# widkyyu/Goal-conditioned-Reinforcement-Learning-with-environmental-and-policy-priors

Hardware: AMD Instinct MI355X
Metric: env-steps/sec (higher is better)
Workload: dtype u8

## Files before the change

goal-conditioned-reinforcement-learning-with-environmental-and-policy-priors_amd/_lib.py:

```python
import ctypes as C
import os
import subprocess

_PKG_DIR = os.path.dirname(os.path.abspath(__file__))
LIB_PATH = os.path.join(_PKG_DIR, "libtwoarmy_hip.so")
CSRC_DIR = os.path.join(_PKG_DIR, "csrc")

TW_CELLS = 289
TW_REC_WORDS = 48
TW_DRAW_WORDS = 8
TW_F_AUTORESET = 1
TW_F_POLICY_IDX = 2
TW_F_MATRIX_CODE = 4
TW_F_SLAB_HIPMALLOC = 8

FIELDS = dict(AX=0, AY=1, DIR=2, STEP_COUNT=3, STEP_MOVE=4, PONE=5, PATROL=6, UP1=7, RIGHT2=8, UPD_LONG=9,
              UPD_HORIZ=10, RISK=11, FIRST_ROOM2=12, OBX=13, OBY=16, O1X=19, O1Y=22, O1_VALID=25, O2X=26,
              O2Y=30, O2_VALID=34, GOAL_X=35, GOAL_Y=36, T=37, ERROR=38, MAX_STEPS=39, EPISODES=40,
              LAST_REWARD=41, LAST_TERM=42, LAST_TRUNC=43, WALL_I1=44, WALL_I2=45)

LAUNCH_FIELDS = ("pipelined", "PG", "LAYOUT", "pipe_grid", "E", "FAST", "seq_grid", "T")

ENV_ERRORS = {1: AttributeError, 2: AssertionError, 3: TypeError}

# ... 105 lines not shown
    "mg_nav_path_scan": (C.c_int, [_vp, _i64, _i, _i, _i, _i, _vp, _vp, _vp, _vp, _vp, _vp, _i, _vp, _vp, _vp, _vp, _vp, _vp,
                                   _vp, _vp, _vp]),
    "mg_nav_path_summary_workspace": (C.c_int, [_i, _i]),
    "mg_nav_path_summary": (C.c_int, [_vp, _vp, _vp, _vp, _vp, _vp, _i, _i, _vp, _vp, _vp]),
    "ppo_her_relabel": (C.c_int, [_vp, _vp, _vp, _vp, _vp, _vp, _u64, C.c_uint32, C.c_uint32, _i, _i, _i, _vp, _vp, _vp,
                                  _vp, _vp, _vp, _vp, _vp]),
    "ppo_her_relabel_window": (C.c_int, [_vp, _vp, _vp, _vp, _vp, _vp, _u64, C.c_uint32, C.c_uint32, _i, _i, _i, _i, _vp,
                                         _vp, _vp, _vp, _vp, _vp, _vp, _vp]),
    "ppo_lstm_cell": (C.c_int, [_vp, _vp, C.c_longlong, _vp, _vp, _vp, _i, _i, _vp]),
    "ppo_decoder_frames": (C.c_int, [_vp, _i, _vp, _vp, _vp, _vp, _vp, C.c_float, _vp, _vp]),
    "ppo_gather_stack_u8": (C.c_int, [_vp, _i, _vp, _i, _vp, _vp, _vp, _vp, _vp, _i, _vp, _vp, _vp]),
    "ppo_age_scan": (C.c_int, [_vp, _vp, _vp, _i, _i, _vp, _vp]),
    "ppo_episode_scan": (C.c_int, [_vp, _vp, _vp, _i, _i, _vp, _vp, _vp, _vp, _vp]),
    "ppo_episode_summary": (C.c_int, [_vp, _vp, _vp, _vp, _vp, _vp, _i, _i, _i, C.c_double, C.c_double, _vp, _vp, _vp, _vp,
                                      _vp, _vp]),
    "ppo_episode_summary_workspace": (C.c_int, [_i, _i]),
    "ppo_visit_scan": (C.c_int, [_vp, _vp, _vp, _i, _i, _i, _i, _vp, _vp, _vp, _vp]),
    "ppo_visit_carry_words": (C.c_int, [_i, _i, _i]),
    "ppo_visit_hist": (C.c_int, [_vp, _i, _i, _vp, _vp, _vp, _i, _i, _i, _vp, _vp]),
    "ppo_bonus_table_words": (C.c_int, [_i, _i, _i, _i, _i, _i]),
    "ppo_bonus_workspace_bytes": (_i64, [_i, _i, _i, _i, _i, _i]),
    "ppo_bonus_scan": (C.c_int, [_vp, _vp, _vp, C.c_long, C.c_long, _vp, _vp, _i, _i, _i, _i, _i, _i, _i, C.c_double, _vp, _vp,
                                 _vp, _vp, _vp, _vp, _vp]),
    "ppo_bonus_episode_words": (C.c_int, [_i, _i, _i, _i, _i]),
    "ppo_bonus_scan_episode": (C.c_int, [_vp, _vp, _vp, C.c_long, C.c_long, _vp, _vp, _vp, _vp, _i, _i, _i, _i, _i, _i, _i,
                                         C.c_double, _vp, _vp, _vp, _vp, _vp, _vp]),
    "ppo_bias_relu_nhwc": (C.c_int, [_vp, _vp, _i64, _i, _vp]),
    "ppo_conv1_up4_bias_relu": (C.c_int, [_vp, _i, _i, _vp, _vp, _vp, _vp]),
    "ppo_conv1_up4_bias_relu_c": (C.c_int, [_vp, _i, _i, _i, _vp, _vp, _vp, _vp]),
    "ppo_conv1_up4_bwd_groups": (C.c_int, [_i]),
    "ppo_conv1_up4_bwd": (C.c_int, [_vp, _i, _i, _vp, _vp, _vp, _vp, _vp]),
    "ppo_relu_bwd_bias_grad_nhwc_blocks": (C.c_int, [_i64, _i]),
    "ppo_relu_bwd_bias_grad_nhwc": (C.c_int, [_vp, _vp, _vp, _vp, _i64, _i, _vp]),
})

_lib = None


def exported_symbols():
    return sorted(_SIGS)


def lib():
    global _lib
    if _lib is None:
        if not os.path.exists(LIB_PATH):
            raise TwoarmyLibraryError(
                "%s not built: run `python -c 'import __graft_entry__ as g; g.build()'` "
                "(hipcc --offload-arch=gfx950); there is no CPU fallback" % LIB_PATH)
        import torch
        try:
            h = C.CDLL(LIB_PATH)
        except OSError as ex:
            raise TwoarmyLibraryError("cannot load %s: %s" % (LIB_PATH, ex)) from ex
        for name, (res, args) in _SIGS.items():
            try:
                fn = getattr(h, name)
            except AttributeError as ex:
                raise TwoarmyLibraryError("%s lacks symbol %s" % (LIB_PATH, name)) from ex
            fn.restype, fn.argtypes = res, args
        runtimes = set()
        try:
            with open("/proc/self/maps") as f:
                for line in f:
                    if "libamdhip64" in line:
                        runtimes.add(line.split()[-1])
# ... 17 lines not shown
```

goal-conditioned-reinforcement-learning-with-environmental-and-policy-priors_amd/csrc/ppo_kernels.hip:

```cpp

#include <hip/hip_runtime.h>
#include <float.h>
#include <stdint.h>

#include <type_traits>

#include "launch.h"
#include "philox.h"
#include "twoarmy.h"
#include "twoarmy_ppo.h"

namespace {

constexpr float CAT_EPS = FLT_EPSILON;

template <int A> __device__ __forceinline__ float cat_row(const float *__restrict__ row, float (&p)[A]) {
    float S = 0.f;
#pragma unroll
    for (int k = 0; k < A; ++k) { p[k] = row[k]; S += p[k]; }
    return S;
}
__device__ __forceinline__ float cat_log(float q) { return logf(fminf(fmaxf(q, CAT_EPS), 1.0f - CAT_EPS)); }

template <typename T, int K> __device__ __forceinline__ void block_sum(T (&v)[K], T *lds) {
    const int tid = threadIdx.x;
#pragma unroll
    for (int k = 0; k < K; ++k) lds[k * 256 + tid] = v[k];
    __syncthreads();
    for (int s = 128; s > 0; s >>= 1) {
        if (tid < s) {
#pragma unroll
            for (int k = 0; k < K; ++k) lds[k * 256 + tid] += lds[k * 256 + tid + s];
        }
        __syncthreads();
    }
#pragma unroll
    for (int k = 0; k < K; ++k) v[k] = lds[k * 256];
}

__device__ __forceinline__ float4 relu4(float4 v) {
    return make_float4(fmaxf(v.x, 0.f), fmaxf(v.y, 0.f), fmaxf(v.z, 0.f), fmaxf(v.w, 0.f));
}
__device__ __forceinline__ float4 mask4(float4 g, float4 y) {
    return make_float4(y.x > 0.f ? g.x : 0.f, y.y > 0.f ? g.y : 0.f, y.z > 0.f ? g.z : 0.f, y.w > 0.f ? g.w : 0.f);
}
__device__ __forceinline__ void add4(float4 &acc, const float4 &o) { acc.x += o.x; acc.y += o.y; acc.z += o.z; acc.w += o.w; }
__device__ __forceinline__ float4 fma4(float x, float4 w, float4 acc) {
    return make_float4(fmaf(x, w.x, acc.x), fmaf(x, w.y, acc.y), fmaf(x, w.z, acc.z), fmaf(x, w.w, acc.w));
}

__device__ __forceinline__ float4 slot_sum4(const float4 *red, int rows, int stride, int cq) {
    float4 sum = red[cq];
    for (int r = 1; r < rows; ++r) add4(sum, red[r * stride + cq]);
    return sum;
}

__device__ __forceinline__ uint32_t done_at(const uint8_t *__restrict__ terminated, const uint8_t *__restrict__ truncated,
                                            size_t i) {
    return (uint32_t)(terminated[i] | truncated[i]);
}

template <int A>
__global__ void ppo_sample_kernel(const float *__restrict__ probs, int B, const float *__restrict__ uniforms,
                                  uint32_t k0, uint32_t k1, uint64_t offset, const uint64_t *__restrict__ offset_dev,
                                  int32_t *__restrict__ action, float *__restrict__ logp) {
    const int b = blockIdx.x * blockDim.x + threadIdx.x;
    if (b >= B) return;
    float p[A];
    const float sum = cat_row<A>(probs + (size_t)b * A, p);
    float u;
    if (uniforms) u = uniforms[b];
    else {
        const uint64_t ctr = (uint64_t)b + offset + (offset_dev ? *offset_dev : 0ull);
        uint32_t c0 = (uint32_t)ctr, c1 = (uint32_t)(ctr >> 32), c2 = 0, c3 = 0x54574F53u;
        philox4x32_10(k0, k1, c0, c1, c2, c3);
        u = (float)(c0 >> 8) * (1.0f / 16777216.0f);
    }
    int a = A - 1, last = A - 1;
    float cum = 0.f, qa = 0.f;
    bool found = false;
#pragma unroll
    for (int k = 0; k < A; ++k) {
        const float q = p[k] / sum;
        cum += q;
        if (q > 0.f) last = k;
        if (!found && cum > u) { a = k; found = true; }
    }
    if (!found) a = last;
#pragma unroll
    for (int k = 0; k < A; ++k) if (k == a) qa = p[k] / sum;
    action[b] = a;
    logp[b] = cat_log(qa);
}

__global__ __launch_bounds__(256) void ppo_bias_relu_kernel(float4 *__restrict__ y, const float4 *__restrict__ bias,
                                                            size_t n4, int c4) {
    const size_t stride = (size_t)gridDim.x * blockDim.x;
    for (size_t i = (size_t)blockIdx.x * blockDim.x + threadIdx.x; i < n4; i += stride) {
        float4 v = y[i];
        add4(v, bias[i % c4]);
        y[i] = relu4(v);
    }
}

__global__ __launch_bounds__(256) void ppo_relu_bwd_bias_grad_kernel(const float4 *__restrict__ gy,
                                                                     const float4 *__restrict__ y,
                                                                     float4 *__restrict__ gx,
                                                                     float4 *__restrict__ partial, size_t n_pixels,
                                                                     int c4, int pixels_per_block) {
    __shared__ float4 red[256];
    const int rows = 256 / c4;
    const int cq = threadIdx.x % c4, row = threadIdx.x / c4;
    const size_t p0 = (size_t)blockIdx.x * pixels_per_block;
    const size_t p1 = p0 + pixels_per_block < n_pixels ? p0 + pixels_per_block : n_pixels;
    float4 acc = make_float4(0.f, 0.f, 0.f, 0.f);
    if (row < rows) {
        for (size_t px = p0 + row; px < p1; px += rows) {
            const size_t i = px * c4 + cq;
            const float4 o = mask4(gy[i], y[i]);
            gx[i] = o;
            add4(acc, o);
        }
    }
    red[threadIdx.x] = acc;
    __syncthreads();
    if (row == 0) partial[(size_t)blockIdx.x * c4 + cq] = slot_sum4(red, rows, c4, cq);
}

template <int F> __device__ __forceinline__ void conv1_stage_frame(float *xs, const float *__restrict__ src, int tid) {
    for (int i = tid; i < F * 324; i += 256) {
        const int c = i / 324, r = i - c * 324, y = r / 18, x = r - y * 18;
        xs[i] = (y < 17 && x < 17) ? src[c * 289 + y * 17 + x] : 0.f;
    }
}

template <int F, int CQ>
__global__ __launch_bounds__(256) void ppo_conv1_up4_kernel(const float *__restrict__ frames, const float4 *__restrict__ wf,
                                                            const float4 *__restrict__ bias, float4 *__restrict__ out, int B) {
    __shared__ float xs[F * 18 * 18];
    constexpr int SLOTS = 256 / CQ;
    const int b = blockIdx.x, tid = threadIdx.x;
    const int cq = tid % CQ, slot = tid / CQ;
    conv1_stage_frame<F>(xs, frames + (size_t)b * F * 289, tid);
    __syncthreads();
    const float4 bv = bias[cq];
    float4 *dst = out + (size_t)b * 1089 * CQ;
#pragma unroll 1
    for (int ph = 0; ph < 4; ++ph) {
        const int py = ph >> 1, px = ph & 1;
        float4 w[4 * F];
#pragma unroll
        for (int k = 0; k < 4 * F; ++k) w[k] = wf[(ph * 4 * F + k) * CQ + cq];
        const int ny = 17 - py, nx = 17 - px;
        for (int q = slot; q < ny * nx; q += SLOTS) {
            const int m = q / nx, n = q - m * nx;
            float4 acc = bv;
#pragma unroll
            for (int t = 0; t < 4; ++t) {
                const int ty = t >> 1, tx = t & 1;
#pragma unroll
                for (int c = 0; c < F; ++c) acc = fma4(xs[c * 324 + (m + ty) * 18 + n + tx], w[t * F + c], acc);
            }
            dst[((2 * m + py) * 33 + 2 * n + px) * CQ + cq] = relu4(acc);
        }
    }
}

template <int F>
__global__ __launch_bounds__(256) void ppo_conv1_up4_bwd_kernel(const float *__restrict__ frames, const float4 *__restrict__ gy,
                                                                const float4 *__restrict__ y, float4 *__restrict__ gw_part,
                                                                float4 *__restrict__ gb_part, int B) {
    __shared__ float xs[F * 18 * 18];
    __shared__ float4 red[256];
    const int tid = threadIdx.x, cq = tid & 15, slot = tid >> 4;
    const int ph = blockIdx.y, py = ph >> 1, px = ph & 1;
    const int ny = 17 - py, nx = 17 - px;
    float4 acc[4 * F];
#pragma unroll
    for (int k = 0; k < 4 * F; ++k) acc[k] = make_float4(0.f, 0.f, 0.f, 0.f);
    float4 accb = make_float4(0.f, 0.f, 0.f, 0.f);
    for (int b = blockIdx.x; b < B; b += gridDim.x) {
        __syncthreads();
        conv1_stage_frame<F>(xs, frames + (size_t)b * F * 289, tid);
        __syncthreads();
        const size_t base = (size_t)b * 1089 * 16;
        for (int q = slot; q < ny * nx; q += 16) {
            const int m = q / nx, n = q - m * nx;
            const size_t o = base + (size_t)((2 * m + py) * 33 + 2 * n + px) * 16 + cq;
            const float4 g = mask4(gy[o], y[o]);
            add4(accb, g);
#pragma unroll
            for (int t = 0; t < 4; ++t) {
                const int ty = t >> 1, tx = t & 1;
#pragma unroll
                for (int c = 0; c < F; ++c) acc[t * F + c] = fma4(xs[c * 324 + (m + ty) * 18 + n + tx], g, acc[t * F + c]);
            }
        }
    }
    const size_t wbase = ((size_t)blockIdx.x * 4 + ph) * (4 * F) * 16;
#pragma unroll
    for (int k = 0; k <= 4 * F; ++k) {
        __syncthreads();
        red[tid] = k < 4 * F ? acc[k < 4 * F ? k : 0] : accb;
        __syncthreads();
        if (slot == 0) {
            const float4 sum = slot_sum4(red, 16, 16, cq);
            if (k < 4 * F) gw_part[wbase + (size_t)k * 16 + cq] = sum;
            else gb_part[((size_t)blockIdx.x * 4 + ph) * 16 + cq] = sum;
        }
    }
}

constexpr int GT = 64;

template <int GN>
__global__ __launch_bounds__(256) void ppo_gae_kernel(const float *__restrict__ reward, const float *__restrict__ value,
                                                      const float *__restrict__ next_value,
                                                      const uint8_t *__restrict__ done, float gamma, float lambda,
                                                      int use_done_mask, int T, int N, float *__restrict__ adv,
                                                      float *__restrict__ target, float *__restrict__ ret) {
    __shared__ float sd[GT][GN + 1];
    __shared__ float sc[GT][GN + 1];
// ... 1156 lines not shown
    if (!all_set(reward, terminated, truncated, carry_return, carry_length) || T <= 0 || N <= 0 ||
        !ep_count_ok((int64_t)T * N) || !aligned_natural(reward, carry_return, carry_length, ep_return, ep_length))
        return TW_E_ARG;
    hipLaunchKernelGGL(ppo_episode_scan_kernel, dim3(blocks(N, 64)), dim3(64), 0, (hipStream_t)stream, reward, terminated,
                       truncated, T, N, carry_return, carry_length, ep_return, ep_length);
    return tw_launched(__func__);
}

int ppo_episode_summary_workspace(int T, int N) {
    if (T <= 0 || N <= 0 || !ep_count_ok((int64_t)T * N)) return TW_E_ARG;
    return ep_summary_blocks((int64_t)T * N) * EP_NV;
}

int ppo_episode_summary(const double *ep_return, const int32_t *ep_length, const uint8_t *terminated,
                        const uint8_t *truncated, const float *reward, const int32_t *action, int A, int T, int N,
                        double keep, double gain, double *score, double *summary, int64_t *action_hist,
                        int64_t *reward_hist, double *workspace, void *stream) {
    if (!all_set(ep_return, ep_length, terminated, truncated, reward, summary, reward_hist, workspace) || T <= 0 || N <= 0 ||
        !ppo_actions_ok(A) || !ep_count_ok((int64_t)T * N) ||
        !aligned_natural(ep_return, ep_length, reward, action, score, summary, action_hist, reward_hist, workspace))
        return TW_E_ARG;
    const int64_t M = (int64_t)T * N;
    const int nblocks = ep_summary_blocks(M);
    const int64_t per_block = (M + nblocks - 1) / nblocks;
    const int per_thread = blocks(per_block, 256);
    hipStream_t st = (hipStream_t)stream;
    hipLaunchKernelGGL(ppo_episode_partial_kernel, dim3(nblocks), dim3(256), 0, st, ep_return, ep_length, terminated,
                       truncated, reward, action, M, per_block, per_thread, keep, gain, workspace);
    hipLaunchKernelGGL(ppo_episode_finalize_kernel, dim3(1), dim3(64), 0, st, workspace, nblocks, A, score, summary,
                       action_hist, reward_hist);
    return tw_launched(__func__);
}

int ppo_bias_relu_nhwc(float *y, const float *bias, int64_t n_pixels, int C, void *stream) {
    if (!all_set(y, bias) || n_pixels <= 0 || C <= 0 || (C & 3) || !aligned16(y, bias)) return TW_E_ARG;
    const size_t n4 = (size_t)n_pixels * (C / 4);
    hipLaunchKernelGGL(ppo_bias_relu_kernel, dim3(blocks_capped((int64_t)n4, 256, 8192)), dim3(256), 0, (hipStream_t)stream,
                       f4(y), f4(bias), n4, C / 4);
    return tw_launched(__func__);
}

int ppo_relu_bwd_bias_grad_nhwc_blocks(int64_t n_pixels, int C) {
    if (n_pixels <= 0 || C <= 0 || (C & 3) || C > 256) return TW_E_ARG;
    return blocks_capped(n_pixels, 512, 4096);
}

int ppo_relu_bwd_bias_grad_nhwc(const float *gy, const float *y, float *gx, float *partial, int64_t n_pixels, int C,
                                void *stream) {
    const int nb = ppo_relu_bwd_bias_grad_nhwc_blocks(n_pixels, C);
    if (nb <= 0 || !all_set(gy, y, gx, partial) || !aligned16(gy, y, gx, partial)) return TW_E_ARG;
    const int ppb = blocks(n_pixels, nb);
    hipLaunchKernelGGL(ppo_relu_bwd_bias_grad_kernel, dim3(nb), dim3(256), 0, (hipStream_t)stream, f4(gy), f4(y), f4(gx),
                       f4(partial), (size_t)n_pixels, C / 4, ppb);
    return tw_launched(__func__);
}

int ppo_conv1_up4_bias_relu(const float *frames, int B, int F, const float *folded_w, const float *bias, float *out,
                            void *stream) {
    return ppo_conv1_up4_bias_relu_c(frames, B, F, 64, folded_w, bias, out, stream);
}

int ppo_conv1_up4_bias_relu_c(const float *frames, int B, int F, int C_out, const float *folded_w, const float *bias,
                              float *out, void *stream) {
    if (!all_set(frames, folded_w, bias, out) || B <= 0 || !aligned16(out, folded_w, bias)) return TW_E_ARG;
    auto launch = [&](auto f, auto cq) {
        hipLaunchKernelGGL((ppo_conv1_up4_kernel<decltype(f)::value, decltype(cq)::value>), dim3(B), dim3(256), 0,
                           (hipStream_t)stream, frames, f4(folded_w), f4(bias), f4(out), B);
    };
    if (F == 4 && C_out == 64) launch(int_c<4>{}, int_c<16>{});
    else if (F == 8 && C_out == 64) launch(int_c<8>{}, int_c<16>{});
    else if (F == 1 && C_out == 16) launch(int_c<1>{}, int_c<4>{});
    else return TW_E_ARG;
    return tw_launched(__func__);
}

int ppo_conv1_up4_bwd_groups(int B) { return B <= 0 ? TW_E_ARG : blocks_capped(B, 1, 256); }

int ppo_conv1_up4_bwd(const float *frames, int B, int F, const float *gy, const float *y, float *gw_partial,
                      float *gb_partial, void *stream) {
    const int groups = ppo_conv1_up4_bwd_groups(B);
    if (groups <= 0 || !all_set(frames, gy, y, gw_partial, gb_partial) || !aligned16(gy, y, gw_partial, gb_partial))
        return TW_E_ARG;
    auto launch = [&](auto f) {
        hipLaunchKernelGGL(ppo_conv1_up4_bwd_kernel<decltype(f)::value>, dim3(groups, 4), dim3(256), 0, (hipStream_t)stream,
                           frames, f4(gy), f4(y), f4(gw_partial), f4(gb_partial), B);
    };
    if (F == 4) launch(int_c<4>{});
    else if (F == 8) launch(int_c<8>{});
    else return TW_E_ARG;
    return tw_launched(__func__);
}

int ppo_decoder_frames(const float *z, int n_frames, const float *w1, const float *b1, const float *w2, const float *b2,
                       const float *kfold, float b3, float *frames, void *stream) {
    if (!all_set(z, w1, b1, w2, b2, kfold, frames) || n_frames <= 0) return TW_E_ARG;
    const int grid = blocks_capped(n_frames, 1, 512);
    hipLaunchKernelGGL(ppo_decoder_frames_kernel, dim3(grid), dim3(256), 0, (hipStream_t)stream, z, n_frames, w1, b1, w2,
                       b2, kfold, b3, frames);
    return tw_launched(__func__);
}

int ppo_lstm_cell(const float *gates_a, const float *gates_b, long long ldb, const float *bias, float *c, float *h, int B,
                  int H, void *stream) {
    if ((!gates_a && !gates_b) || !all_set(c, h) || B <= 0 || H <= 0 || (H & 3) || !aligned16(gates_a, gates_b, bias, c, h))
        return TW_E_ARG;
    if (gates_b && ((ldb & 3) || ldb < 4LL * H)) return TW_E_ARG;
    const long long n = (long long)B * (H / 4);
    if (n > 0x7fffffffLL) return TW_E_ARG;
    hipLaunchKernelGGL(ppo_lstm_cell_kernel, dim3(blocks(n, 256)), dim3(256), 0, (hipStream_t)stream, f4(gates_a),
                       f4(gates_b), ldb / 4, f4(bias), f4(c), f4(h), B, H / 4);
    return tw_launched(__func__);
}

}
```

goal-conditioned-reinforcement-learning-with-environmental-and-policy-priors_amd/ppo_ops.py:

```python
import ctypes as C

import torch

from ._marshal import call as _call, constant as _constant, ptr as _p, query as _query

_CL = torch.channels_last


def _pf(t):
    return _p(t.detach().contiguous(), torch.float32)


def _step_outputs(out, want_steps, T, N, dtypes, device):
    if out is None:
        return tuple(torch.empty((T, N), dtype=d, device=device) if want_steps else None for d in dtypes)
    assert out[0].shape == (T, N) and out[1].shape == (T, N)
    return out


def sample(probs, uniforms=None, seed=0, offset=0, offset_dev=None):
    B, A = probs.shape
    action = torch.empty(B, dtype=torch.int32, device=probs.device)
    logp = torch.empty(B, dtype=torch.float32, device=probs.device)
    _call("ppo_sample_dev", probs, _p(probs, torch.float32), B, A, _p(uniforms, torch.float32), seed, offset,
# ... 274 lines not shown
                                   lambda kind, N: bonus_episode_words(kind, width, height, n_actions, N))
    _call("ppo_bonus_scan_episode", pos, _p(pos, torch.float32), _p(action, torch.int32), *dirs,
          _p(reward, torch.float32), _p(keep, torch.uint8), _p(terminated, torch.uint8), _p(truncated, torch.uint8), T, N,
          int(width), int(height), int(n_actions), mask, BONUS_FORMS[form], float(scale), _p(state_table, torch.int32),
          _p(action_table, torch.int32), _p(bonus_state, torch.float32), _p(bonus_action, torch.float32),
          _p(reward_out, torch.float32))
    return reward_out


def her_relabel(pos, terminated, truncated, age0, reward, choices=None, seed=0, env_id0=0, step0=0, max_goals=4, skip=0):
    T, N = terminated.shape
    dev = pos.device
    assert pos.shape == (T, N, 2) and pos.is_contiguous() and reward.shape == (T, N)
    if choices is not None:
        assert choices.shape == (T, N, 4) and choices.dtype == torch.int32 and choices.is_contiguous()
    counts = torch.empty(N, dtype=torch.int32, device=dev)
    args = [_p(pos, torch.float32), _p(terminated.contiguous(), torch.uint8), _p(truncated.contiguous(), torch.uint8),
            _p(age0.contiguous(), torch.int32), _p(reward.contiguous(), torch.float32), _p(choices), int(seed),
            int(env_id0), int(step0), T, N, int(max_goals), int(skip)]
    _call("ppo_her_relabel_window", pos, *args, None, _p(counts), None, None, None, None, None)
    incl = torch.cumsum(counts.long(), 0)
    H = int(incl[-1])
    offsets = (incl - counts.long()).contiguous()
    out = dict(t=torch.empty(H, dtype=torch.int32, device=dev), n=torch.empty(H, dtype=torch.int32, device=dev),
               goal=torch.empty((H, 2), dtype=torch.float32, device=dev),
               reward=torch.empty(H, dtype=torch.float32, device=dev), done=torch.empty(H, dtype=torch.uint8, device=dev),
               counts=counts)
    if H:
        _call("ppo_her_relabel_window", pos, *args, _p(offsets), _p(counts), _p(out["t"]), _p(out["n"]), _p(out["goal"]),
              _p(out["reward"]), _p(out["done"]))
    return out


class _ConvBiasReLU(torch.autograd.Function):

    @staticmethod
    def forward(ctx, x, w, b, stride):
        y = torch.ops.aten.convolution(x, w, None, list(stride), [0, 0], [1, 1], False, [0, 0], 1)
        assert y.is_contiguous(memory_format=torch.channels_last), "conv epilogue kernels need channels-last activations"
        B, Cc, H, W = y.shape
        _call("ppo_bias_relu_nhwc", y, _p(y, None, _CL), _pf(b), B * H * W, Cc)
        ctx.save_for_backward(x, w, y)
        ctx.stride = list(stride)
        return y

    @staticmethod
    def backward(ctx, gy):
        x, w, y = ctx.saved_tensors
        gy = gy.contiguous(memory_format=torch.channels_last)
        B, Cc, H, W = y.shape
        npix = B * H * W
        blocks = _query("ppo_relu_bwd_bias_grad_nhwc_blocks", npix, Cc)
        g = torch.empty_like(y)
        partial = torch.empty((blocks, Cc), dtype=torch.float32, device=y.device)
        _call("ppo_relu_bwd_bias_grad_nhwc", y, _p(gy, None, _CL), _p(y, None, _CL), _p(g, None, _CL), _p(partial), npix, Cc)
        gx, gw, _ = torch.ops.aten.convolution_backward(g, x, w, None, ctx.stride, [0, 0], [1, 1], False, [0, 0], 1,
                                                        [bool(ctx.needs_input_grad[0]), True, False])
        return gx, gw, partial.sum(0), None


def conv_bias_relu(x, weight, bias, stride):
    assert x.is_cuda and x.dtype == torch.float32 and x.is_contiguous(memory_format=torch.channels_last)
    return _ConvBiasReLU.apply(x, weight, bias, tuple(stride))


def fold_conv1_weights(w):
    O, F = w.shape[0], w.shape[1]
    w = w.detach().reshape(O, F, 4, 4).float()
    z = torch.zeros_like(w[:, :, 0:1, :])
    rows = torch.stack([torch.cat([w.sum(2, keepdim=True), z], 2),
                        torch.cat([w[:, :, 0:2].sum(2, keepdim=True), w[:, :, 2:4].sum(2, keepdim=True)], 2)], 0)
    zc = torch.zeros_like(rows[..., 0:1])
    cols = torch.stack([torch.cat([rows.sum(-1, keepdim=True), zc], -1),
                        torch.cat([rows[..., 0:2].sum(-1, keepdim=True), rows[..., 2:4].sum(-1, keepdim=True)], -1)], 1)
    return cols.permute(0, 1, 4, 5, 3, 2).contiguous()


@torch.no_grad()
def conv1_up4_bias_relu_infer(frames, weight, bias):
    B, F, _ = frames.shape
    Cout = weight.shape[0]
    y = torch.empty((B, Cout, 33, 33), dtype=torch.float32, device=frames.device, memory_format=torch.channels_last)
    wf = fold_conv1_weights(weight)
    _call("ppo_conv1_up4_bias_relu_c", y, _pf(frames), B, F, Cout, _p(wf), _pf(bias), _p(y, None, _CL))
    return y


class _Conv1Up4(torch.autograd.Function):

    @staticmethod
    def forward(ctx, frames, w, b, wf):
        B, F, _ = frames.shape
        y = torch.empty((B, w.shape[0], 33, 33), dtype=torch.float32, device=frames.device,
                        memory_format=torch.channels_last)
        if wf is None:
            wf = fold_conv1_weights(w)
        fr = frames.contiguous()
        _call("ppo_conv1_up4_bias_relu", y, _p(fr, torch.float32), B, F, _p(wf), _pf(b), _p(y, None, _CL))
        ctx.save_for_backward(fr, w, y)
        return y

    @staticmethod
    def backward(ctx, gy):
        fr, w, y = ctx.saved_tensors
        gy = gy.contiguous(memory_format=torch.channels_last)
        B, F = fr.shape[0], fr.shape[1]
        groups = _query("ppo_conv1_up4_bwd_groups", B)
        gw_part = torch.empty((groups, 2, 2, 2, 2, F, 64), dtype=torch.float32, device=y.device)
        gb_part = torch.empty((groups, 4, 64), dtype=torch.float32, device=y.device)
        _call("ppo_conv1_up4_bwd", y, _p(fr, torch.float32), B, F, _p(gy, None, _CL), _p(y, None, _CL), _p(gw_part),
              _p(gb_part))
        return None, unfold_conv1_grad(gw_part.sum(0)).to(w.dtype), gb_part.sum((0, 1)), None


def unfold_conv1_grad(gwf):
    ty = _constant("conv1_tap_of_row", [[0, 0, 0, 0], [0, 0, 1, 1]], torch.int64, gwf.device)
    out = None
    for py in (0, 1):
        for px in (0, 1):
            g = gwf[py, px][ty[py]][:, ty[px]]
            out = g if out is None else out + g
    return out.permute(3, 2, 0, 1).contiguous()


def conv1_up4_bias_relu(frames, weight, bias, folded=None):
    assert frames.is_cuda and frames.dtype == torch.float32 and weight.shape[2:] == (4, 4) and weight.shape[0] == 64
    return _Conv1Up4.apply(frames, weight, bias, folded)


def fold_decoder_tail(w3):
    m = _constant("decoder_tail_rows", [[0., 0., 1., 1.], [1., 1., 1., 1.], [1., 1., 0., 0.]], w3.dtype, w3.device)
    return torch.einsum("ur,crs,vs->cuv", m, w3[:, 0], m).mul_(1.0 / 16.0).contiguous()


def decoder_frames(z, w1, b1, w2, b2, w3, b3):
    assert z.dim() == 4 and tuple(z.shape[1:]) == (64, 4, 4) and z.dtype == torch.float32
    z = z.contiguous()
    n = z.shape[0]
    out = torch.empty((n, 289), dtype=torch.float32, device=z.device)
    if n:
        _call("ppo_decoder_frames", z, _p(z), n, _pf(w1), _pf(b1), _pf(w2), _pf(b2), _p(fold_decoder_tail(w3.detach())), 0.0,
              _p(out))
        out += b3.detach().view(1, 1)
    return out


def lstm_cell_(gates, c, gates_b=None, bias=None):
    B, H = c.shape
    H4 = 4 * H
    assert c.dtype == torch.float32 and (gates is not None or gates_b is not None)
    assert gates is None or (gates.shape == (B, H4) and gates.dtype == torch.float32)
    pb, ldb = None, 0
    if gates_b is not None:
        assert gates_b.shape == (B, H4) and gates_b.stride(1) == 1 and gates_b.dtype == torch.float32 and gates_b.is_cuda
        pb, ldb = C.c_void_p(gates_b.data_ptr()), gates_b.stride(0) if B > 1 else H4
    h = torch.empty_like(c)
    _call("ppo_lstm_cell", c, _p(gates), pb, ldb, _p(bias), _p(c), _p(h), B, H)
    return h
```

include/twoarmy_ppo.h:

```cpp
#ifndef TWOARMY_PPO_H
#define TWOARMY_PPO_H

#include <stdint.h>

#ifdef __cplusplus
extern "C" {
#endif

int ppo_sample(const float *probs, int B, int A, const float *uniforms, uint64_t seed, uint64_t offset,
               int32_t *action, float *logp, void *stream);
int ppo_sample_dev(const float *probs, int B, int A, const float *uniforms, uint64_t seed, uint64_t offset,
                   const uint64_t *offset_dev, int32_t *action, float *logp, void *stream);

int ppo_gae(const float *reward, const float *value, const float *next_value, const uint8_t *done,
            float gamma, float lambda, int use_done_mask, int T, int N, float *adv, float *target, float *ret,
            void *stream);

int ppo_run_ends(const int32_t *t, const int32_t *n, const float *goal, const uint8_t *done, int64_t H,
                 uint8_t *run_end, int32_t *broken, void *stream);
int ppo_gae_runs(const float *reward, const float *value, const float *next_value, const uint8_t *done,
                 const uint8_t *run_end, float gamma, float lambda, int use_done_mask, int64_t H,
                 float *adv, float *target, float *ret, float *workspace, void *stream);
int ppo_gae_runs_workspace(int64_t H);

// ... 50 lines not shown
                   float *bonus_action, float *reward_out, void *workspace, void *stream);

#define BONUS_EPISODE_COUNT_BITS 24
int ppo_bonus_episode_words(int kind, int width, int height, int n_actions, int N);
int ppo_bonus_scan_episode(const float *pos, const int32_t *action, const int32_t *dir, long dir_stride_t, long dir_stride_n,
                           const float *reward, const uint8_t *keep, const uint8_t *terminated, const uint8_t *truncated,
                           int T, int N, int width, int height, int n_actions, int kind_mask, int form, double scale,
                           void *state_table, void *action_table, float *bonus_state, float *bonus_action,
                           float *reward_out, void *stream);

int ppo_her_relabel(const float *pos, const uint8_t *terminated, const uint8_t *truncated, const int32_t *age0,
                    const float *reward, const int32_t *choices, uint64_t seed, uint32_t env_id0, uint32_t step0, int T,
                    int N, int max_goals, const int64_t *offsets, int32_t *counts, int32_t *out_t, int32_t *out_n,
                    float *out_goal, float *out_reward, uint8_t *out_done, void *stream);
int ppo_her_relabel_window(const float *pos, const uint8_t *terminated, const uint8_t *truncated, const int32_t *age0,
                           const float *reward, const int32_t *choices, uint64_t seed, uint32_t env_id0, uint32_t step0,
                           int T, int N, int max_goals, int skip, const int64_t *offsets, int32_t *counts, int32_t *out_t,
                           int32_t *out_n, float *out_goal, float *out_reward, uint8_t *out_done, void *stream);

int ppo_bias_relu_nhwc(float *y, const float *bias, int64_t n_pixels, int C, void *stream);
int ppo_relu_bwd_bias_grad_nhwc_blocks(int64_t n_pixels, int C);
int ppo_relu_bwd_bias_grad_nhwc(const float *gy, const float *y, float *gx, float *partial, int64_t n_pixels, int C,
                                void *stream);

int ppo_conv1_up4_bias_relu(const float *frames, int B, int F, const float *folded_w, const float *bias, float *out,
                            void *stream);
int ppo_conv1_up4_bias_relu_c(const float *frames, int B, int F, int C_out, const float *folded_w, const float *bias,
                              float *out, void *stream);

int ppo_conv1_up4_bwd_groups(int B);
int ppo_conv1_up4_bwd(const float *frames, int B, int F, const float *gy, const float *y, float *gw_partial,
                      float *gb_partial, void *stream);

int ppo_decoder_frames(const float *z, int n_frames, const float *w1, const float *b1, const float *w2, const float *b2,
                       const float *kfold, float b3, float *frames, void *stream);

int ppo_lstm_cell(const float *gates_a, const float *gates_b, long long ldb, const float *bias, float *c, float *h, int B,
                  int H, void *stream);

#ifdef __cplusplus
}
#endif
#endif
```

Baseline: 2.871 billion.

## Save ReLU activations as packed bitmasks for backward instead of full fp32 outputs

Forward conv epilogue kernels now wavefront-ballot the ReLU sign bits and write a packed 1-bit-per-element mask. Autograd saves that mask instead of the fp32 activation, and the backward kernels read the bits to gate gradients. This cuts backward memory traffic and saved-activation footprint, at the cost of extra ballot and store work in forward. The saved y may still be kept alive by downstream layers, so the memory saving is not guaranteed.

```diff
diff --git a/goal-conditioned-reinforcement-learning-with-environmental-and-policy-priors_amd/_lib.py b/goal-conditioned-reinforcement-learning-with-environmental-and-policy-priors_amd/_lib.py
--- a/goal-conditioned-reinforcement-learning-with-environmental-and-policy-priors_amd/_lib.py
+++ b/goal-conditioned-reinforcement-learning-with-environmental-and-policy-priors_amd/_lib.py
@@ -161,6 +161,11 @@
     "ppo_conv1_up4_bwd": (C.c_int, [_vp, _i, _i, _vp, _vp, _vp, _vp, _vp]),
     "ppo_relu_bwd_bias_grad_nhwc_blocks": (C.c_int, [_i64, _i]),
     "ppo_relu_bwd_bias_grad_nhwc": (C.c_int, [_vp, _vp, _vp, _vp, _i64, _i, _vp]),
+    "ppo_relu_mask_words": (_i64, [_i64, _i]),
+    "ppo_bias_relu_nhwc_bits": (C.c_int, [_vp, _vp, _i64, _i, _vp, _i64, _vp]),
+    "ppo_relu_bwd_bias_grad_nhwc_bits": (C.c_int, [_vp, _vp, _i64, _vp, _vp, _i64, _i, _vp]),
+    "ppo_conv1_up4_bias_relu_bits": (C.c_int, [_vp, _i, _i, _vp, _vp, _vp, _vp, _i64, _vp]),
+    "ppo_conv1_up4_bwd_bits": (C.c_int, [_vp, _i, _i, _vp, _vp, _i64, _vp, _vp, _vp]),
 })
 
 _lib = None
diff --git a/goal-conditioned-reinforcement-learning-with-environmental-and-policy-priors_amd/csrc/ppo_kernels.hip b/goal-conditioned-reinforcement-learning-with-environmental-and-policy-priors_amd/csrc/ppo_kernels.hip
--- a/goal-conditioned-reinforcement-learning-with-environmental-and-policy-priors_amd/csrc/ppo_kernels.hip
+++ b/goal-conditioned-reinforcement-learning-with-environmental-and-policy-priors_amd/csrc/ppo_kernels.hip
@@ -44,6 +44,34 @@
 __device__ __forceinline__ float4 mask4(float4 g, float4 y) {
     return make_float4(y.x > 0.f ? g.x : 0.f, y.y > 0.f ? g.y : 0.f, y.z > 0.f ? g.z : 0.f, y.w > 0.f ? g.w : 0.f);
 }
+
+struct ballots {
+    uint64_t x, y, z, w;
+    __device__ __forceinline__ uint64_t of(int j) const { return j == 0 ? x : j == 1 ? y : j == 2 ? z : w; }
+};
+__device__ __forceinline__ ballots ballot4(float4 v) {
+    return ballots{__ballot(v.x > 0.f), __ballot(v.y > 0.f), __ballot(v.z > 0.f), __ballot(v.w > 0.f)};
+}
+__device__ __forceinline__ uint32_t mask_word(const ballots b, int c4, int k) {
+    if (c4 == 16) {
+        const int s = (k >> 1) * 16, j = (k & 1) * 2;
+        return (uint32_t)((b.of(j) >> s) & 0xffffu) | ((uint32_t)((b.of(j + 1) >> s) & 0xffffu) << 16);
+    }
+    if (c4 == 32) return (uint32_t)(b.of(k & 3) >> ((k >> 2) * 32));
+    return (uint32_t)(b.of(k >> 1) >> ((k & 1) * 32));
+}
+struct relu_of_y {
+    const float4 *__restrict__ y;
+    __device__ __forceinline__ float4 operator()(float4 g, size_t px, int c4, int cq) const { return mask4(g, y[px * c4 + cq]); }
+};
+struct relu_of_bits {
+    const uint32_t *__restrict__ bits;
+    __device__ __forceinline__ float4 operator()(float4 g, size_t px, int c4, int cq) const {
+        const uint32_t *w = bits + px * (size_t)(c4 >> 3);
+        const auto on = [&](int j) { const int t = j * c4 + cq; return (w[t >> 5] >> (t & 31)) & 1u; };
+        return make_float4(on(0) ? g.x : 0.f, on(1) ? g.y : 0.f, on(2) ? g.z : 0.f, on(3) ? g.w : 0.f);
+    }
+};
 __device__ __forceinline__ void add4(float4 &acc, const float4 &o) { acc.x += o.x; acc.y += o.y; acc.z += o.z; acc.w += o.w; }
 __device__ __forceinline__ float4 fma4(float x, float4 w, float4 acc) {
     return make_float4(fmaf(x, w.x, acc.x), fmaf(x, w.y, acc.y), fmaf(x, w.z, acc.z), fmaf(x, w.w, acc.w));
@@ -93,18 +121,26 @@
     logp[b] = cat_log(qa);
 }
 
+template <bool BITS>
 __global__ __launch_bounds__(256) void ppo_bias_relu_kernel(float4 *__restrict__ y, const float4 *__restrict__ bias,
-                                                            size_t n4, int c4) {
+                                                            size_t n4, int c4, uint32_t *__restrict__ bits) {
     const size_t stride = (size_t)gridDim.x * blockDim.x;
     for (size_t i = (size_t)blockIdx.x * blockDim.x + threadIdx.x; i < n4; i += stride) {
         float4 v = y[i];
         add4(v, bias[i % c4]);
-        y[i] = relu4(v);
-    }
-}
-
-__global__ __launch_bounds__(256) void ppo_relu_bwd_bias_grad_kernel(const float4 *__restrict__ gy,
-                                                                     const float4 *__restrict__ y,
+        v = relu4(v);
+        y[i] = v;
+        if constexpr (BITS) {
+            const ballots b = ballot4(v);
+            const int lane = threadIdx.x & 63;
+            const size_t word = (i - lane) / 8 + lane;
+            if (lane < 8 && word < n4 / 8) bits[word] = mask_word(b, c4, lane);
+        }
+    }
+}
+
+template <typename Relu>
+__global__ __launch_bounds__(256) void ppo_relu_bwd_bias_grad_kernel(const float4 *__restrict__ gy, const Relu relu,
                                                                      float4 *__restrict__ gx,
                                                                      float4 *__restrict__ partial, size_t n_pixels,
                                                                      int c4, int pixels_per_block) {
@@ -117,7 +153,7 @@
     if (row < rows) {
         for (size_t px = p0 + row; px < p1; px += rows) {
             const size_t i = px * c4 + cq;
-            const float4 o = mask4(gy[i], y[i]);
+            const float4 o = relu(gy[i], px, c4, cq);
             gx[i] = o;
             add4(acc, o);
         }
@@ -134,9 +170,11 @@
     }
 }
 
-template <int F, int CQ>
+template <int F, int CQ, bool BITS>
 __global__ __launch_bounds__(256) void ppo_conv1_up4_kernel(const float *__restrict__ frames, const float4 *__restrict__ wf,
-                                                            const float4 *__restrict__ bias, float4 *__restrict__ out, int B) {
+                                                            const float4 *__restrict__ bias, float4 *__restrict__ out, int B,
+                                                            uint32_t *__restrict__ bits) {
+    static_assert(!BITS || CQ == 16, "the mask layout needs whole 32-bit words per pixel");
     __shared__ float xs[F * 18 * 18];
     constexpr int SLOTS = 256 / CQ;
     const int b = blockIdx.x, tid = threadIdx.x;
@@ -161,14 +199,20 @@
 #pragma unroll
                 for (int c = 0; c < F; ++c) acc = fma4(xs[c * 324 + (m + ty) * 18 + n + tx], w[t * F + c], acc);
             }
-            dst[((2 * m + py) * 33 + 2 * n + px) * CQ + cq] = relu4(acc);
-        }
-    }
-}
-
-template <int F>
+            const int pix = (2 * m + py) * 33 + 2 * n + px;
+            const float4 v = relu4(acc);
+            dst[pix * CQ + cq] = v;
+            if constexpr (BITS) {
+                const ballots bal = ballot4(v);
+                if (cq < 2) bits[((size_t)b * 1089 + pix) * 2 + cq] = mask_word(bal, 16, ((tid & 63) >> 4) * 2 + cq);
+            }
+        }
+    }
+}
+
+template <int F, typename Relu>
 __global__ __launch_bounds__(256) void ppo_conv1_up4_bwd_kernel(const float *__restrict__ frames, const float4 *__restrict__ gy,
-                                                                const float4 *__restrict__ y, float4 *__restrict__ gw_part,
+                                                                const Relu relu, float4 *__restrict__ gw_part,
                                                                 float4 *__restrict__ gb_part, int B) {
     __shared__ float xs[F * 18 * 18];
     __shared__ float4 red[256];
@@ -183,11 +227,11 @@
         __syncthreads();
         conv1_stage_frame<F>(xs, frames + (size_t)b * F * 289, tid);
         __syncthreads();
-        const size_t base = (size_t)b * 1089 * 16;
+        const size_t base = (size_t)b * 1089;
         for (int q = slot; q < ny * nx; q += 16) {
             const int m = q / nx, n = q - m * nx;
-            const size_t o = base + (size_t)((2 * m + py) * 33 + 2 * n + px) * 16 + cq;
-            const float4 g = mask4(gy[o], y[o]);
+            const size_t pix = base + (size_t)((2 * m + py) * 33 + 2 * n + px);
+            const float4 g = relu(gy[pix * 16 + cq], pix, 16, cq);
             add4(accb, g);
 #pragma unroll
             for (int t = 0; t < 4; ++t) {
@@ -1410,63 +1454,143 @@
     return tw_launched(__func__);
 }
 
-int ppo_bias_relu_nhwc(float *y, const float *bias, int64_t n_pixels, int C, void *stream) {
-    if (!all_set(y, bias) || n_pixels <= 0 || C <= 0 || (C & 3) || !aligned16(y, bias)) return TW_E_ARG;
-    const size_t n4 = (size_t)n_pixels * (C / 4);
-    hipLaunchKernelGGL(ppo_bias_relu_kernel, dim3(blocks_capped((int64_t)n4, 256, 8192)), dim3(256), 0, (hipStream_t)stream,
-                       f4(y), f4(bias), n4, C / 4);
-    return tw_launched(__func__);
-}
-
 int ppo_relu_bwd_bias_grad_nhwc_blocks(int64_t n_pixels, int C) {
     if (n_pixels <= 0 || C <= 0 || (C & 3) || C > 256) return TW_E_ARG;
     return blocks_capped(n_pixels, 512, 4096);
 }
 
-int ppo_relu_bwd_bias_grad_nhwc(const float *gy, const float *y, float *gx, float *partial, int64_t n_pixels, int C,
-                                void *stream) {
+int ppo_conv1_up4_bwd_groups(int B) { return B <= 0 ? TW_E_ARG : blocks_capped(B, 1, 256); }
+
+int64_t ppo_relu_mask_words(int64_t n_pixels, int C) {
+    if (n_pixels <= 0 || (C != 64 && C != 128 && C != 256) || !ep_count_ok(n_pixels)) return TW_E_ARG;
+    return n_pixels * (C / 32);
+}
+
+}
+
+namespace {
+struct mask_arg { bool given = false; uint32_t *words = nullptr; int64_t n_words = 0; };
+mask_arg mask_of(const uint32_t *words, int64_t n_words) { return mask_arg{true, const_cast<uint32_t *>(words), n_words}; }
+bool mask_ok(const mask_arg &m, int64_t n_pixels, int C) {
+    if (!m.given) return true;
+    const int64_t need = ppo_relu_mask_words(n_pixels, C);
+    return m.words && aligned16(m.words) && need > 0 && m.n_words >= need;
+}
+
+int bias_relu(const char *what, float *y, const float *bias, int64_t n_pixels, int C, mask_arg m, void *stream) {
+    if (!all_set(y, bias) || n_pixels <= 0 || C <= 0 || (C & 3) || !aligned16(y, bias) || !mask_ok(m, n_pixels, C))
+        return TW_E_ARG;
+    const size_t n4 = (size_t)n_pixels * (C / 4);
+    auto launch = [&](auto bits) {
+        hipLaunchKernelGGL(ppo_bias_relu_kernel<decltype(bits)::value>, dim3(blocks_capped((int64_t)n4, 256, 8192)), dim3(256),
+                           0, (hipStream_t)stream, f4(y), f4(bias), n4, C / 4, m.words);
+    };
+    if (m.given) launch(std::true_type{});
+    else launch(std::false_type{});
+    return tw_launched(what);
+}
+
+int relu_bwd_bias_grad(const char *what, const float *gy, const float *y, mask_arg m, float *gx, float *partial,
+                       int64_t n_pixels, int C, void *stream) {
     const int nb = ppo_relu_bwd_bias_grad_nhwc_blocks(n_pixels, C);
-    if (nb <= 0 || !all_set(gy, y, gx, partial) || !aligned16(gy, y, gx, partial)) return TW_E_ARG;
+    if (nb <= 0 || !all_set(gy, gx, partial) || (!m.given && !y) || !aligned16(gy, y, gx, partial) || !mask_ok(m, n_pixels, C))
+        return TW_E_ARG;
     const int ppb = blocks(n_pixels, nb);
-    hipLaunchKernelGGL(ppo_relu_bwd_bias_grad_kernel, dim3(nb), dim3(256), 0, (hipStream_t)stream, f4(gy), f4(y), f4(gx),
-                       f4(partial), (size_t)n_pixels, C / 4, ppb);
-    return tw_launched(__func__);
-}
-
-int ppo_conv1_up4_bias_relu(const float *frames, int B, int F, const float *folded_w, const float *bias, float *out,
-                            void *stream) {
-    return ppo_conv1_up4_bias_relu_c(frames, B, F, 64, folded_w, bias, out, stream);
-}
-
-int ppo_conv1_up4_bias_relu_c(const float *frames, int B, int F, int C_out, const float *folded_w, const float *bias,
-                              float *out, void *stream) {
-    if (!all_set(frames, folded_w, bias, out) || B <= 0 || !aligned16(out, folded_w, bias)) return TW_E_ARG;
+    auto launch = [&](auto relu) {
+        hipLaunchKernelGGL(ppo_relu_bwd_bias_grad_kernel<decltype(relu)>, dim3(nb), dim3(256), 0, (hipStream_t)stream, f4(gy),
+                           relu, f4(gx), f4(partial), (size_t)n_pixels, C / 4, ppb);
+    };
+    if (m.given) launch(relu_of_bits{m.words});
+    else launch(relu_of_y{f4(y)});
+    return tw_launched(what);
+}
+
+int conv1_up4(const char *what, const float *frames, int B, int F, int C_out, const float *folded_w, const float *bias,
+              float *out, mask_arg m, void *stream) {
+    if (!all_set(frames, folded_w, bias, out) || B <= 0 || !aligned16(out, folded_w, bias) ||
+        !mask_ok(m, (int64_t)B * 1089, C_out))
+        return TW_E_ARG;
     auto launch = [&](auto f, auto cq) {
-        hipLaunchKernelGGL((ppo_conv1_up4_kernel<decltype(f)::value, decltype(cq)::value>), dim3(B), dim3(256), 0,
-                           (hipStream_t)stream, frames, f4(folded_w), f4(bias), f4(out), B);
+        constexpr int Fv = decltype(f)::value, CQ = decltype(cq)::value;
+        auto go = [&](auto bits) {
+            hipLaunchKernelGGL((ppo_conv1_up4_kernel<Fv, CQ, decltype(bits)::value>), dim3(B), dim3(256), 0, (hipStream_t)stream,
+                               frames, f4(folded_w), f4(bias), f4(out), B, m.words);
+        };
+        if constexpr (CQ == 16) { if (m.given) return go(std::true_type{}); }
+        go(std::false_type{});
     };
     if (F == 4 && C_out == 64) launch(int_c<4>{}, int_c<16>{});
     else if (F == 8 && C_out == 64) launch(int_c<8>{}, int_c<16>{});
     else if (F == 1 && C_out == 16) launch(int_c<1>{}, int_c<4>{});
     else return TW_E_ARG;
-    return tw_launched(__func__);
-}
-
-int ppo_conv1_up4_bwd_groups(int B) { return B <= 0 ? TW_E_ARG : blocks_capped(B, 1, 256); }
+    return tw_launched(what);
+}
+
+int conv1_up4_bwd(const char *what, const float *frames, int B, int F, const float *gy, const float *y, mask_arg m,
+                  float *gw_partial, float *gb_partial, void *stream) {
+    const int groups = ppo_conv1_up4_bwd_groups(B);
+    if (groups <= 0 || !all_set(frames, gy, gw_partial, gb_partial) || (!m.given && !y) ||
+        !aligned16(gy, y, gw_partial, gb_partial) || !mask_ok(m, (int64_t)B * 1089, 64))
+        return TW_E_ARG;
+    auto launch = [&](auto f, auto relu) {
+        hipLaunchKernelGGL((ppo_conv1_up4_bwd_kernel<decltype(f)::value, decltype(relu)>), dim3(groups, 4), dim3(256), 0,
+                           (hipStream_t)stream, frames, f4(gy), relu, f4(gw_partial), f4(gb_partial), B);
+    };
+    auto with_relu = [&](auto f) {
+        if (m.given) launch(f, relu_of_bits{m.words});
+        else launch(f, relu_of_y{f4(y)});
+    };
+    if (F == 4) with_relu(int_c<4>{});
+    else if (F == 8) with_relu(int_c<8>{});
+    else return TW_E_ARG;
+    return tw_launched(what);
+}
+}
+
+extern "C" {
+
+int ppo_bias_relu_nhwc(float *y, const float *bias, int64_t n_pixels, int C, void *stream) {
+    return bias_relu(__func__, y, bias, n_pixels, C, mask_arg{}, stream);
+}
+
+int ppo_bias_relu_nhwc_bits(float *y, const float *bias, int64_t n_pixels, int C, uint32_t *mask, int64_t mask_words,
+                            void *stream) {
+    return bias_relu(__func__, y, bias, n_pixels, C, mask_of(mask, mask_words), stream);
+}
+
+int ppo_relu_bwd_bias_grad_nhwc(const float *gy, const float *y, float *gx, float *partial, int64_t n_pixels, int C,
+                                void *stream) {
+    return relu_bwd_bias_grad(__func__, gy, y, mask_arg{}, gx, partial, n_pixels, C, stream);
+}
+
+int ppo_relu_bwd_bias_grad_nhwc_bits(const float *gy, const uint32_t *mask, int64_t mask_words, float *gx, float *partial,
+                                     int64_t n_pixels, int C, void *stream) {
+    return relu_bwd_bias_grad(__func__, gy, nullptr, mask_of(mask, mask_words), gx, partial, n_pixels, C, stream);
+}
+
+int ppo_conv1_up4_bias_relu(const float *frames, int B, int F, const float *folded_w, const float *bias, float *out,
+                            void *stream) {
+    return conv1_up4(__func__, frames, B, F, 64, folded_w, bias, out, mask_arg{}, stream);
+}
+
+int ppo_conv1_up4_bias_relu_c(const float *frames, int B, int F, int C_out, const float *folded_w, const float *bias,
+                              float *out, void *stream) {
+    return conv1_up4(__func__, frames, B, F, C_out, folded_w, bias, out, mask_arg{}, stream);
+}
+
+int ppo_conv1_up4_bias_relu_bits(const float *frames, int B, int F, const float *folded_w, const float *bias, float *out,
+                                 uint32_t *mask, int64_t mask_words, void *stream) {
+    return conv1_up4(__func__, frames, B, F, 64, folded_w, bias, out, mask_of(mask, mask_words), stream);
+}
 
 int ppo_conv1_up4_bwd(const float *frames, int B, int F, const float *gy, const float *y, float *gw_partial,
                       float *gb_partial, void *stream) {
-    const int groups = ppo_conv1_up4_bwd_groups(B);
-    if (groups <= 0 || !all_set(frames, gy, y, gw_partial, gb_partial) || !aligned16(gy, y, gw_partial, gb_partial))
-        return TW_E_ARG;
-    auto launch = [&](auto f) {
-        hipLaunchKernelGGL(ppo_conv1_up4_bwd_kernel<decltype(f)::value>, dim3(groups, 4), dim3(256), 0, (hipStream_t)stream,
-                           frames, f4(gy), f4(y), f4(gw_partial), f4(gb_partial), B);
-    };
-    if (F == 4) launch(int_c<4>{});
-    else if (F == 8) launch(int_c<8>{});
-    else return TW_E_ARG;
-    return tw_launched(__func__);
+    return conv1_up4_bwd(__func__, frames, B, F, gy, y, mask_arg{}, gw_partial, gb_partial, stream);
+}
+
+int ppo_conv1_up4_bwd_bits(const float *frames, int B, int F, const float *gy, const uint32_t *mask, int64_t mask_words,
+                           float *gw_partial, float *gb_partial, void *stream) {
+    return conv1_up4_bwd(__func__, frames, B, F, gy, nullptr, mask_of(mask, mask_words), gw_partial, gb_partial, stream);
 }
 
 int ppo_decoder_frames(const float *z, int n_frames, const float *w1, const float *b1, const float *w2, const float *b2,
diff --git a/goal-conditioned-reinforcement-learning-with-environmental-and-policy-priors_amd/ppo_ops.py b/goal-conditioned-reinforcement-learning-with-environmental-and-policy-priors_amd/ppo_ops.py
--- a/goal-conditioned-reinforcement-learning-with-environmental-and-policy-priors_amd/ppo_ops.py
+++ b/goal-conditioned-reinforcement-learning-with-environmental-and-policy-priors_amd/ppo_ops.py
@@ -330,36 +330,63 @@
     return out
 
 
+MASK_CHANNELS = (64, 128, 256)
+RELU_MASK_BITS = True
+
+
+def _wants_mask(C, *tensors):
+    return RELU_MASK_BITS and C in MASK_CHANNELS and torch.is_grad_enabled() and any(t.requires_grad for t in tensors)
+
+
+def _new_mask(npix, C, device):
+    return torch.empty(_query("ppo_relu_mask_words", npix, C), dtype=torch.int32, device=device)
+
+
+def unpack_relu_mask(mask, npix, C):
+    words = mask[:npix * C // 32].reshape(npix, C // 32, 1)
+    bits = (words >> torch.arange(32, dtype=torch.int32, device=mask.device)) & 1
+    return bits.reshape(npix, 4, C // 4).permute(0, 2, 1).reshape(npix, C).bool()
+
+
 class _ConvBiasReLU(torch.autograd.Function):
 
     @staticmethod
-    def forward(ctx, x, w, b, stride):
+    def forward(ctx, x, w, b, stride, bits):
         y = torch.ops.aten.convolution(x, w, None, list(stride), [0, 0], [1, 1], False, [0, 0], 1)
         assert y.is_contiguous(memory_format=torch.channels_last), "conv epilogue kernels need channels-last activations"
         B, Cc, H, W = y.shape
-        _call("ppo_bias_relu_nhwc", y, _p(y, None, _CL), _pf(b), B * H * W, Cc)
-        ctx.save_for_backward(x, w, y)
-        ctx.stride = list(stride)
+        if bits:
+            mask = _new_mask(B * H * W, Cc, y.device)
+            _call("ppo_bias_relu_nhwc_bits", y, _p(y, None, _CL), _pf(b), B * H * W, Cc, _p(mask), mask.numel())
+        else:
+            _call("ppo_bias_relu_nhwc", y, _p(y, None, _CL), _pf(b), B * H * W, Cc)
+        ctx.save_for_backward(x, w, mask if bits else y)
+        ctx.stride, ctx.bits = list(stride), bits
         return y
 
     @staticmethod
     def backward(ctx, gy):
-        x, w, y = ctx.saved_tensors
+        x, w, saved = ctx.saved_tensors
         gy = gy.contiguous(memory_format=torch.channels_last)
-        B, Cc, H, W = y.shape
+        B, Cc, H, W = gy.shape
         npix = B * H * W
         blocks = _query("ppo_relu_bwd_bias_grad_nhwc_blocks", npix, Cc)
-        g = torch.empty_like(y)
-        partial = torch.empty((blocks, Cc), dtype=torch.float32, device=y.device)
-        _call("ppo_relu_bwd_bias_grad_nhwc", y, _p(gy, None, _CL), _p(y, None, _CL), _p(g, None, _CL), _p(partial), npix, Cc)
+        g = torch.empty_like(gy)
+        partial = torch.empty((blocks, Cc), dtype=torch.float32, device=gy.device)
+        if ctx.bits:
+            _call("ppo_relu_bwd_bias_grad_nhwc_bits", gy, _p(gy, None, _CL), _p(saved, torch.int32), saved.numel(),
+                  _p(g, None, _CL), _p(partial), npix, Cc)
+        else:
+            _call("ppo_relu_bwd_bias_grad_nhwc", gy, _p(gy, None, _CL), _p(saved, None, _CL), _p(g, None, _CL), _p(partial),
+                  npix, Cc)
         gx, gw, _ = torch.ops.aten.convolution_backward(g, x, w, None, ctx.stride, [0, 0], [1, 1], False, [0, 0], 1,
                                                         [bool(ctx.needs_input_grad[0]), True, False])
-        return gx, gw, partial.sum(0), None
+        return gx, gw, partial.sum(0), None, None
 
 
 def conv_bias_relu(x, weight, bias, stride):
     assert x.is_cuda and x.dtype == torch.float32 and x.is_contiguous(memory_format=torch.channels_last)
-    return _ConvBiasReLU.apply(x, weight, bias, tuple(stride))
+    return _ConvBiasReLU.apply(x, weight, bias, tuple(stride), _wants_mask(weight.shape[0], x, weight, bias))
 
 
 def fold_conv1_weights(w):
@@ -387,28 +414,38 @@
 class _Conv1Up4(torch.autograd.Function):
 
     @staticmethod
-    def forward(ctx, frames, w, b, wf):
+    def forward(ctx, frames, w, b, wf, bits):
         B, F, _ = frames.shape
         y = torch.empty((B, w.shape[0], 33, 33), dtype=torch.float32, device=frames.device,
                         memory_format=torch.channels_last)
         if wf is None:
             wf = fold_conv1_weights(w)
         fr = frames.contiguous()
-        _call("ppo_conv1_up4_bias_relu", y, _p(fr, torch.float32), B, F, _p(wf), _pf(b), _p(y, None, _CL))
-        ctx.save_for_backward(fr, w, y)
+        if bits:
+            mask = _new_mask(B * 1089, 64, y.device)
+            _call("ppo_conv1_up4_bias_relu_bits", y, _p(fr, torch.float32), B, F, _p(wf), _pf(b), _p(y, None, _CL), _p(mask),
+                  mask.numel())
+        else:
+            _call("ppo_conv1_up4_bias_relu", y, _p(fr, torch.float32), B, F, _p(wf), _pf(b), _p(y, None, _CL))
+        ctx.save_for_backward(fr, w, mask if bits else y)
+        ctx.bits = bits
         return y
 
     @staticmethod
     def backward(ctx, gy):
-        fr, w, y = ctx.saved_tensors
+        fr, w, saved = ctx.saved_tensors
         gy = gy.contiguous(memory_format=torch.channels_last)
         B, F = fr.shape[0], fr.shape[1]
         groups = _query("ppo_conv1_up4_bwd_groups", B)
-        gw_part = torch.empty((groups, 2, 2, 2, 2, F, 64), dtype=torch.float32, device=y.device)
-        gb_part = torch.empty((groups, 4, 64), dtype=torch.float32, device=y.device)
-        _call("ppo_conv1_up4_bwd", y, _p(fr, torch.float32), B, F, _p(gy, None, _CL), _p(y, None, _CL), _p(gw_part),
-              _p(gb_part))
-        return None, unfold_conv1_grad(gw_part.sum(0)).to(w.dtype), gb_part.sum((0, 1)), None
+        gw_part = torch.empty((groups, 2, 2, 2, 2, F, 64), dtype=torch.float32, device=gy.device)
+        gb_part = torch.empty((groups, 4, 64), dtype=torch.float32, device=gy.device)
+        if ctx.bits:
+            _call("ppo_conv1_up4_bwd_bits", gy, _p(fr, torch.float32), B, F, _p(gy, None, _CL), _p(saved, torch.int32),
+                  saved.numel(), _p(gw_part), _p(gb_part))
+        else:
+            _call("ppo_conv1_up4_bwd", gy, _p(fr, torch.float32), B, F, _p(gy, None, _CL), _p(saved, None, _CL), _p(gw_part),
+                  _p(gb_part))
+        return None, unfold_conv1_grad(gw_part.sum(0)).to(w.dtype), gb_part.sum((0, 1)), None, None
 
 
 def unfold_conv1_grad(gwf):
@@ -423,7 +460,7 @@
 
 def conv1_up4_bias_relu(frames, weight, bias, folded=None):
     assert frames.is_cuda and frames.dtype == torch.float32 and weight.shape[2:] == (4, 4) and weight.shape[0] == 64
-    return _Conv1Up4.apply(frames, weight, bias, folded)
+    return _Conv1Up4.apply(frames, weight, bias, folded, _wants_mask(64, weight, bias))
 
 
 def fold_decoder_tail(w3):
diff --git a/include/twoarmy_ppo.h b/include/twoarmy_ppo.h
--- a/include/twoarmy_ppo.h
+++ b/include/twoarmy_ppo.h
@@ -106,6 +106,16 @@
 int ppo_conv1_up4_bwd(const float *frames, int B, int F, const float *gy, const float *y, float *gw_partial,
                       float *gb_partial, void *stream);
 
+int64_t ppo_relu_mask_words(int64_t n_pixels, int C);
+int ppo_bias_relu_nhwc_bits(float *y, const float *bias, int64_t n_pixels, int C, uint32_t *mask, int64_t mask_words,
+                            void *stream);
+int ppo_relu_bwd_bias_grad_nhwc_bits(const float *gy, const uint32_t *mask, int64_t mask_words, float *gx, float *partial,
+                                     int64_t n_pixels, int C, void *stream);
+int ppo_conv1_up4_bias_relu_bits(const float *frames, int B, int F, const float *folded_w, const float *bias, float *out,
+                                 uint32_t *mask, int64_t mask_words, void *stream);
+int ppo_conv1_up4_bwd_bits(const float *frames, int B, int F, const float *gy, const uint32_t *mask, int64_t mask_words,
+                           float *gw_partial, float *gb_partial, void *stream);
+
 int ppo_decoder_frames(const float *z, int n_frames, const float *w1, const float *b1, const float *w2, const float *b2,
                        const float *kfold, float b3, float *frames, void *stream);
 
```

Result: no change. 2.873 billion, median of 3 (+0.1%).
